# rgl-epfl/unbiased-inverse-volume-rendering

Hardware: AMD Instinct MI355X
Metric: Msamples/s primal+adjoint DRT, 256^3 grid 512^2x32spp (higher is better)
Workload: dtype f32; 1 GPU; dust-devil 256^3 sigma_t+albedo, 512x512x32spp, volpathsimple-drt, max_depth 64, majorant_resolution_factor 8 (the reference default, scene_config.py:36; with --full the global majorant is reported under other_configs.headline_global_majorant), single sensor, image tiles sharded over 1 GPU(s); spp=32, integrator=volpathsimple-drt

## Files before the change

unbiased-inverse-volume-rendering_amd/csrc/drt_capi.cpp:

```cpp
#include "../../include/drt_hip.h"
#include "drt_launch.h"

#include <hip/hip_runtime.h>

#include <cstdarg>
#include <cstdio>
#include <cmath>
#include <cstdlib>
#include <cstring>
#include <new>
#include <string>
#include <utility>
#include <vector>

using namespace drt;

#ifndef DRT_PATH_CACHE_CAP
#define DRT_PATH_CACHE_CAP 64
#endif
#ifndef DRT_ORDER_ITERS
#define DRT_ORDER_ITERS 1
#endif
#ifndef DRT_SQ_UNIT_EMPTY
#define DRT_SQ_UNIT_EMPTY 1
// ... 10 lines not shown

enum AllocMode { kMust, kBestEffort };
struct DevBuf {
    void *p = nullptr;
    size_t bytes = 0;
    DevBuf() = default;
    DevBuf(const DevBuf &) = delete;
    DevBuf &operator=(const DevBuf &) = delete;
    ~DevBuf() { release(); }
    template <class T> T *as() const { return (T *) p; }
    void release() { if (p) (void) hipFree(p); p = nullptr; bytes = 0; }
    int resize(drt_handle h, size_t need, AllocMode mode, bool wait_side = false, bool pretend_no_memory = false);
    int grow(drt_handle h, size_t need, AllocMode mode) { return need <= bytes ? DRT_OK : resize(h, need, mode); }
};

struct drt_handle_s {
    int device = 0;
    hipStream_t stream = nullptr;
    drt_config cfg{};
    drt::Params base{};
    bool have_medium = false, have_emitter = false, have_sensor = false;
    int32_t phase_kind = DRT_PHASE_ISOTROPIC;
    float *d_majorant = nullptr;
    float *h_majorant = nullptr;
    hipEvent_t ev_majorant = nullptr;
    bool majorant_pending = false;
    float majorant_seen = -1.0f;
    uint32_t *d_scratch = nullptr;
    unsigned long long *d_counters = nullptr;
    DevBuf gt;
    unsigned long long *d_queues = nullptr;
    DevBuf sq_cold;
    DevBuf uempty;
    DevBuf order;
    uint64_t order_first = 0, order_end = 0;
    uint32_t order_unit = 0;
    DevBuf tail;
    int n_cus = 256;
    DevBuf sigma_b;
    uint32_t *d_occ = nullptr;
    DevBuf mgrid;
    float *d_env = nullptr;
    DevBuf grid4;
    uint64_t grid4_version = 0;
    uint64_t medium_version = 0;
    struct RecSlot {
        DevBuf mem;
        uint64_t rays = 0;
        int bins = 0;
        bool tiny = false;
        uint32_t per_ray[2] = {0, 0};
        drt::DeferredPlan plan{};
        size_t clear_bytes = 0;
        hipEvent_t traced = nullptr, reduced = nullptr;
        bool busy = false;
    } rec[2];
    hipStream_t side = nullptr;
    const drt::DeferredPlan *early_plan = nullptr;
    bool early_done = false;
    bool early_partition = false;
    DevBuf sq_tail;
    hipEvent_t ev_split = nullptr, ev_hist = nullptr;
    hipStream_t nerf_stream = nullptr;
    hipEvent_t ev_fork = nullptr, ev_join = nullptr;
    DevBuf loss_partials;
    DevBuf dl_px;
// ... 309 lines not shown
    return DRT_OK;
}

int launch_coop(drt_handle h, const drt::Params &P, bool adjoint)
{
    drt::Params PT = P;
    no_tail(PT);
    const bool tail_pays = P.n_rays - P.ray_first >= (3u << 19) || dbg(h->debug_flags, kHookScheduleSmall);
    if (adjoint && !P.mgrid && P.n_rays > P.ray_first && tail_pays) {
        const size_t want = (((size_t) (P.n_rays - P.ray_first) / 8 + 255) / 256) * 256;
        DRT_TRY(h->tail.grow(h, want ? 256 + want * 128 : 0, kBestEffort));
        if (h->tail.p && want >= 256) {
            PT.tail_count = h->tail.as<uint32_t>(); PT.tail_pool = (uint4 *) (h->tail.as<char>() + 256); PT.tail_cap = (uint32_t) want;
        }
    }
    if (P.mgrid) {
        drt::Params Q = PT;
        Q.ray_perm = nullptr;
        DRT_HIP_CHECK(h, drt::launch_trace_coop(Q, drt::Phase::kIso, adjoint, h->counting, h->stream));
        return DRT_OK;
    }
    const bool early = adjoint && h->early_plan && PT.rec_buf[0] && PT.tail_pool && !dbg(h->debug_flags, kHookNoTailOverlap);
    if (early) {
        DRT_TRY(ensure_side_stream(h));
        DRT_TRY(ensure_event_pair(h, h->ev_split, h->ev_hist));
    }
    EarlyCtx ctx{ h, &PT };
    bool called = false;
    DRT_HIP_CHECK(h, drt::launch_trace_coop(PT, drt::Phase::kIso, adjoint, h->counting, h->stream, early ? early_histogram_between : nullptr, &ctx, &called));
    h->early_done = called;
    return DRT_OK;
}

int bind_unit_empty(drt_handle h, const drt::Params &P, drt::Params &Q)
{
    const uint64_t span = P.n_rays - P.ray_first;
    if (!(DRT_SQ_UNIT_EMPTY && P.sensor_flow && P.mocc && P.spp && span < (1ull << 31) && P.ray_first % P.spp == 0 &&
          P.ray_offset % P.spp == 0 && P.chunk % P.spp == 0 && P.stride % P.spp == 0 && !dbg(h->debug_flags, kHookWalkEmptyPixels)))
        return DRT_OK;
    const uint32_t eunits = (uint32_t) ((span + P.spp - 1) / P.spp);
    DRT_TRY(h->uempty.grow(h, eunits, kBestEffort));
    if (h->uempty.p) {
        DRT_HIP_CHECK(h, drt::build_unit_empty(P, P.spp, eunits, h->uempty.as<uint8_t>(), h->stream));
        Q.unit_empty = h->uempty.as<const uint8_t>(); Q.empty_unit = P.spp;
    }
    return DRT_OK;
}

int bind_ray_order(drt_handle h, const drt::Params &P, drt::Params &Q, bool adjoint, bool iters_ok)
{
    const uint64_t span = P.n_rays - P.ray_first;
    const uint32_t unit = P.spp >= 4u ? P.spp : 16u;
    const uint64_t min_span = dbg(h->debug_flags, kHookScheduleSmall) ? 4096u : (1u << 20);
    if (!(span >= min_span && span < (1ull << 31) && unit <= 256u && !dbg(h->debug_flags, kHookIndexOrder))) return DRT_OK;
    const uint32_t units = (uint32_t) ((span + unit - 1) / unit);
    const size_t need = drt::super_order_bytes(units);
    if (need > h->order.bytes) {
        h->order_unit = 0;
        DRT_TRY(h->order.resize(h, need, kBestEffort));
    }
    if (!h->order.p) return DRT_OK;
    const uint8_t *iters = (DRT_ORDER_ITERS && adjoint && P.path_cache_mode == 2 && iters_ok) ? P.ray_iters : nullptr;
    const bool reuse = !iters && adjoint && P.path_cache_mode == 2 && h->order_unit == unit && h->order_first == P.ray_first && h->order_end == P.n_rays;
    if (!reuse) DRT_HIP_CHECK(h, drt::build_super_order(P, unit, units, h->order.p, h->stream, iters));
    h->order_unit = (!adjoint && P.path_cache_mode == 1) || reuse ? unit : 0u;
    h->order_first = P.ray_first; h->order_end = P.n_rays;
    Q.order = h->order.as<const uint32_t>(); Q.order_unit = unit; Q.order_units = units;
    return DRT_OK;
}

int begin_supergrid_launch(drt_handle h, const drt::Params &P, drt::Params &Q, bool adjoint, const Choice &c)
{
    Q.queues = h->d_queues;
    DRT_TRY(bind_ray_order(h, P, Q, adjoint, c.route == Route::kQueued));
    Q.ray_perm = nullptr; Q.block_order = nullptr;
    if (h->majorant_pending && hipEventQuery(h->ev_majorant) == hipSuccess) { h->majorant_seen = *h->h_majorant; h->majorant_pending = false; }
    else if (h->majorant_pending) (void) hipGetLastError();
    const float dx = P.bmax[0] - P.bmin[0], dy = P.bmax[1] - P.bmin[1], dz = P.bmax[2] - P.bmin[2];
    Q.sq_rounds = (c.phase == drt::Phase::kIso && !adjoint && h->majorant_seen >= 0.0f && h->majorant_seen * std::sqrt(dx * dx + dy * dy + dz * dz) < 3.0f) ? 1u : 0u;
    DRT_HIP_CHECK(h, hipMemsetAsync(h->d_queues, 0, 8 * sizeof(unsigned long long), h->stream));
    return DRT_OK;
}

int bind_sq_tail(drt_handle h, drt::Params &Q, bool adjoint, bool hg, bool *big)
{
    const uint64_t span = Q.n_rays - Q.ray_first;
    const uint64_t tail_min = dbg(h->debug_flags, kHookScheduleSmall) ? 4096u : (1u << 21);
    *big = adjoint && h->early_plan && Q.rec_buf[0] && span >= tail_min;
    const bool solo = drt::sq_tail_solo(Q) && span >= 8192u && !*big &&
                      (adjoint ? ((DRT_SQ_TAIL_SOLO & 2) != 0 && Q.rec_buf[0] != nullptr) : (DRT_SQ_TAIL_SOLO & 1) != 0);
    const bool tail = !hg && DRT_SQ_TAIL && (*big || solo) && !dbg(h->debug_flags, kHookNoTailOverlap) && (DRT_SQ_TAIL_THIN || !Q.sq_rounds);
    if (!tail) return DRT_OK;
    const size_t cap = (size_t) h->n_cus * drt::sq_tail_push();
    DRT_TRY(h->sq_tail.grow(h, 256 + cap * drt::sq_tail_entry_quads() * sizeof(uint4), kBestEffort));
    if (!h->sq_tail.p) return DRT_OK;
    DRT_HIP_CHECK(h, hipMemsetAsync(h->sq_tail.p, 0, 256, h->stream));
    Q.tail_count = h->sq_tail.as<uint32_t>(); Q.tail_pool = (uint4 *) (h->sq_tail.as<char>() + 256); Q.tail_cap = (uint32_t) cap; Q.tail_mode = 0;
    return DRT_OK;
}

int launch_queued(drt_handle h, const drt::Params &P, bool adjoint, const Choice &c)
{
    drt::Params Q = P;
    if (adjoint && P.dL_pix) {
        const uint64_t px = (P.n_rays + P.spp - 1) / P.spp;
        DRT_TRY(h->dl_px.grow(h, (size_t) px * P.spp * 3 * sizeof(float), kMust));
        DRT_HIP_CHECK(h, drt::launch_film_backward(P.dL_pix, px, P.spp, h->dl_px.as<float>(), h->stream));
        Q.dL = h->dl_px.as<float>(); Q.dL_pix = nullptr;
    }
    DRT_TRY(bind_unit_empty(h, P, Q));
    DRT_TRY(begin_supergrid_launch(h, P, Q, adjoint, c));
    Q.sq_cold = h->sq_cold.p;
    bool big = false;
    const bool hg = c.phase != drt::Phase::kIso;
    DRT_TRY(bind_sq_tail(h, Q, adjoint, hg, &big));
    if (hg) no_tail(Q);
    DRT_HIP_CHECK(h, drt::launch_trace_sq(Q, c.phase, adjoint, h->counting, h->n_cus, h->stream));
    if (!Q.tail_pool) return DRT_OK;
    if (big) {
        DRT_TRY(ensure_side_stream(h));
        DRT_TRY(ensure_event_pair(h, h->ev_split, h->ev_hist));
        DRT_HIP_CHECK(h, hipEventRecord(h->ev_split, h->stream));
        DRT_HIP_CHECK(h, hipStreamWaitEvent(h->side, h->ev_split, 0));
        TimedSpan span;
        DRT_HIP_CHECK(h, span.begin(h, h->side));
        DRT_HIP_CHECK(h, drt::launch_deferred_reduce(Q, *h->early_plan, h->side, nullptr, false, 1));
        DRT_HIP_CHECK(h, span.end(2));
        DRT_HIP_CHECK(h, hipEventRecord(h->ev_hist, h->side));
    }
    drt::Params T = Q;
    T.tail_mode = big ? 1 : 2;
    if (big) {
        T.rec_cursor = h->sq_tail.as<uint32_t>() + 8;
        T.rec_cap_chunks[0] = T.rec_cap_chunks[1] = 0;
    }
    T.order = nullptr; T.unit_empty = nullptr;
    DRT_HIP_CHECK(h, drt::launch_trace_sq(T, c.phase, adjoint, h->counting, h->n_cus, h->stream));
    if (big) { h->early_done = true; h->early_partition = true; }
    return DRT_OK;
}

#ifdef DRT_TEST_HOOKS
int launch_older(drt_handle h, const drt::Params &P, bool adjoint, const Choice &c)
// ... 255 lines not shown
    }
    *out = h;
    return DRT_OK;
}

int drt_destroy(drt_handle h)
{
    if (!h) return DRT_OK;
    DeviceGuard g(h->device);
    for (void *p : { (void *) h->d_majorant, (void *) h->d_scratch, (void *) h->d_counters, (void *) h->d_queues, (void *) h->d_occ, (void *) h->d_env })
        if (p) (void) hipFree(p);
    if (h->h_majorant) (void) hipHostFree(h->h_majorant);
    for (hipEvent_t e : { h->ev_majorant, h->ev_fork, h->ev_join, h->ev_split, h->ev_hist, h->rec[0].traced, h->rec[0].reduced, h->rec[1].traced, h->rec[1].reduced })
        if (e) (void) hipEventDestroy(e);
    for (hipStream_t st : { h->side, h->nerf_stream })
        if (st) (void) hipStreamDestroy(st);
    clear_timings(h);
    delete h;
    return DRT_OK;
}

int drt_release_scratch(drt_handle h)
{
    if (!h) return fail(nullptr, DRT_ERR_INVALID_ARGUMENT, "null handle");
    DeviceGuard g(h->device);
    DRT_HIP_CHECK(h, hipStreamSynchronize(h->stream));
    if (h->side) DRT_HIP_CHECK(h, hipStreamSynchronize(h->side));
    for (auto &R : h->rec) {
        R.mem.release();
        R.rays = 0; R.bins = 0; R.busy = false;
    }
    h->pcache.release();
    h->pcache_sig.valid = false; h->order_valid = false; h->order_rays = 0;
    h->tail.release();
    h->dl_px.release();
    return DRT_OK;
}

int drt_set_stream(drt_handle h, void *hip_stream)
{
    if (!h) return fail(nullptr, DRT_ERR_INVALID_ARGUMENT, "null handle");
    h->stream = (hipStream_t) hip_stream;
    return DRT_OK;
}

int drt_set_ray_interleave(drt_handle h, uint64_t chunk_rays, uint64_t stride_rays)
{
    if (!h) return fail(nullptr, DRT_ERR_INVALID_ARGUMENT, "null handle");
    if (chunk_rays && stride_rays < chunk_rays)
        return fail(h, DRT_ERR_INVALID_ARGUMENT, "stride_rays must be >= chunk_rays");
    h->chunk = chunk_rays; h->stride = chunk_rays ? stride_rays : 0;
    return DRT_OK;
}

int drt_synchronize(drt_handle h)
{
    if (!h) return fail(nullptr, DRT_ERR_INVALID_ARGUMENT, "null handle");
    DeviceGuard g(h->device);
    DRT_HIP_CHECK(h, hipStreamSynchronize(h->stream));
    return DRT_OK;
}

int drt_params_changed(drt_handle h)
{
    if (!h) return fail(nullptr, DRT_ERR_INVALID_ARGUMENT, "null handle");
    h->scene_version++; h->medium_version++;
// ... 1084 lines not shown
```

unbiased-inverse-volume-rendering_amd/csrc/drt_kernels.hip:

```cpp
#include "drt_device.h"
#include "drt_launch.h"
#include "drt_coop_tracer.h"
#include "drt_nerf_kernel.h"
#include "drt_film.h"

#ifndef DRT_TRACE_WAVES
#define DRT_TRACE_WAVES 4
#endif
#ifndef DRT_XCD_RUN
#define DRT_XCD_RUN 256
#endif
namespace drt {

struct Ray { V3 o, d; float maxt; };
struct Mei { bool valid; float t; V3 p; float sigma_t; };
struct PathState { int depth; Hit si; float last_pdf; bool escaped; bool active; };

#ifdef DRT_TEST_HOOKS
template <bool COUNT, bool ENV, bool DEFER = false>
struct Tracer {
    const Params &P;
    float maj, inv_maj;
    uint32_t ray_index;
    uint32_t *rec;
// ... 634 lines not shown
    const uint32_t r = rl + batch_first * spp;
    uint32_t b = r / spp;
    Pcg32 S0; S0.seed(seed_pixels, b);
    float us = S0.next_1d(), ux = S0.next_1d(), uy = S0.next_1d();
    uint32_t si = (uint32_t)((float) n_sensors * us);
    if (si >= (uint32_t) n_sensors) si = (uint32_t) n_sensors - 1;
    const float *sn = sensors + 16 * si;
    Params P;
#pragma unroll
    for (int k = 0; k < 3; ++k) { P.cam_o[k] = sn[k]; P.cam_left[k] = sn[3 + k]; P.cam_up[k] = sn[6 + k]; P.cam_dir[k] = sn[9 + k]; }
    P.tan_x = sn[12]; P.tan_y = sn[13]; P.width = (int) sn[14]; P.height = (int) sn[15];
    uint32_t px = (uint32_t)((float) P.width * ux), py = (uint32_t)((float) P.height * uy);
    if (r == b * spp) {
        const uint32_t bl = b - batch_first;
        if (sensor_idx) sensor_idx[bl] = si;
        if (pixels) { pixels[2 * bl] = px; pixels[2 * bl + 1] = py; }
    }
    Pcg32 S1; S1.seed(seed_rays, r);
    float ox = S1.next_1d(), oy = S1.next_1d();
    V3 o, d;
    sensor_ray(P, py * (uint32_t) P.width + px, ox, oy, o, d);
    rays_o[3 * (size_t) rl] = o.x; rays_o[3 * (size_t) rl + 1] = o.y; rays_o[3 * (size_t) rl + 2] = o.z;
    rays_d[3 * (size_t) rl] = d.x; rays_d[3 * (size_t) rl + 1] = d.y; rays_d[3 * (size_t) rl + 2] = d.z;
}

__global__ void __launch_bounds__(256) film_develop_kernel(const float *L, uint64_t n_pixels, uint32_t spp, float *image)
{
    uint64_t t = (uint64_t) blockIdx.x * blockDim.x + threadIdx.x;
    if (t >= n_pixels * 3) return;
    uint64_t p = t / 3; uint32_t c = (uint32_t)(t - p * 3);
    image[t] = film_channel_sum(L, p, c, spp) * (1.0f / (float) spp);
}

__global__ void __launch_bounds__(256) film_develop_wave_kernel(const float *L, uint64_t n_pixels, uint32_t spp, float *image)
{
    const uint64_t p = (uint64_t) blockIdx.x * 4 + (threadIdx.x >> 6);
    if (p >= n_pixels) return;
    const uint32_t lane = threadIdx.x & 63u;
    float s0, s1, s2;
    film_wave_sums(L, p, spp, lane, s0, s1, s2);
    if (lane == 0) {
        const float inv = 1.0f / (float) spp;
        image[3 * p] = s0 * inv; image[3 * p + 1] = s1 * inv; image[3 * p + 2] = s2 * inv;
    }
}

__global__ void __launch_bounds__(256) film_backward_kernel(const float *grad_image, uint64_t n_pixels, uint32_t spp, float *dL)
{
    uint64_t t = (uint64_t) blockIdx.x * blockDim.x + threadIdx.x;
    if (t >= n_pixels * spp * 3) return;
    uint64_t i = t / 3; uint32_t c = (uint32_t)(t - i * 3);
    dL[t] = grad_image[3 * (i / spp) + c] * (1.0f / (float) spp);
}

__global__ void __launch_bounds__(256) debug_eval_kernel(const Params P, int op, const float *in, uint64_t n, float *out)
{
    uint64_t i = (uint64_t) blockIdx.x * blockDim.x + threadIdx.x;
    if (i >= n) return;
    const float *a = in + 6 * i;
    float *o = out + 6 * i;
    for (int k = 0; k < 6; ++k) o[k] = 0.0f;
    switch (op) {
        case 0: o[0] = drt_logf(a[0]); break;
        case 1: drt_sincos_2pi(a[0], o[0], o[1]); break;
        case 2: { V3 d = square_to_uniform_sphere(a[0], a[1]); o[0] = d.x; o[1] = d.y; o[2] = d.z; } break;
        case 3: o[0] = eval_sigma_t(P, v3(a[0], a[1], a[2]), P.occ); break;
        case 4: eval_albedo(P, v3(a[0], a[1], a[2]), o); break;
        case 5: {
            Hit h = box_hit(P, v3(a[0], a[1], a[2]), v3(a[3], a[4], a[5]));
            o[0] = h.valid ? 1.0f : 0.0f; o[1] = h.t; o[2] = h.n.x; o[3] = h.n.y; o[4] = h.n.z;
        } break;
        case 6: {
            Pcg32 S; S.seed(__float_as_uint(a[0]), __float_as_uint(a[1]));
            for (int k = 0; k < 6; ++k) o[k] = S.next_1d();
        } break;
        case 7: {
            V3 ro, rd; sensor_ray(P, __float_as_uint(a[0]), a[1], a[2], ro, rd);
            o[0] = ro.x; o[1] = ro.y; o[2] = ro.z; o[3] = rd.x; o[4] = rd.y; o[5] = rd.z;
        } break;
        case 10: o[0] = drt_expf(a[0]); break;
        case 11: o[0] = drt_atan2f(a[0], a[1]); break;
        case 12: if (P.env_pix) {
            V3 d = v3(a[0], a[1], a[2]); float Le[3];
            envmap_eval(P, d, Le); o[0] = Le[0]; o[1] = Le[1]; o[2] = Le[2]; o[3] = envmap_pdf(P, d);
        } break;
// ... 182 lines not shown
                       dim3(kUntileLanes * kUntileRows), 0, stream, P, nc, chunk);
    return hipGetLastError();
}

hipError_t launch_majorant(const float *sigma_t, size_t n, float scale, uint32_t *scratch_bits,
                           float *majorant, hipStream_t stream)
{
    hipError_t e = hipMemsetAsync(scratch_bits, 0, sizeof(uint32_t), stream);
    if (e != hipSuccess) return e;
    unsigned blocks = (unsigned) ((n + 255) / 256);
    if (blocks > 2048) blocks = 2048;
    if (blocks == 0) blocks = 1;
    hipLaunchKernelGGL(majorant_reduce_kernel, dim3(blocks), dim3(256), 0, stream, sigma_t, n, scratch_bits);
    hipLaunchKernelGGL(majorant_finalize_kernel, dim3(1), dim3(1), 0, stream, scratch_bits, scale, majorant);
    return hipGetLastError();
}

hipError_t launch_batch_raygen(const float *sensors, int n_sensors, uint32_t batch_first, uint32_t batch_size, uint32_t spp,
                               uint32_t seed_pixels, uint32_t seed_rays, float *rays_o, float *rays_d, uint32_t *sensor_idx,
                               uint32_t *pixels, hipStream_t stream)
{
    uint64_t n = (uint64_t) batch_size * spp;
    if (n == 0) return hipSuccess;
    hipLaunchKernelGGL(batch_raygen_kernel, dim3((unsigned)((n + 255) / 256)), dim3(256), 0, stream, sensors, n_sensors,
                       batch_first, batch_size, spp, seed_pixels, seed_rays, rays_o, rays_d, sensor_idx, pixels);
    return hipGetLastError();
}

hipError_t launch_film_develop(const float *L, uint64_t n_pixels, uint32_t spp, float *image, hipStream_t stream)
{
    uint64_t n = n_pixels * 3;
    if (n == 0) return hipSuccess;
    if (spp >= kFilmWaveSpp) hipLaunchKernelGGL(film_develop_wave_kernel, dim3((unsigned)((n_pixels + 3) / 4)), dim3(256), 0, stream, L, n_pixels, spp, image);
    else hipLaunchKernelGGL(film_develop_kernel, dim3((unsigned)((n + 255) / 256)), dim3(256), 0, stream, L, n_pixels, spp, image);
    return hipGetLastError();
}

__global__ void __launch_bounds__(256) adam_step_kernel(float *p, const float *g, float *m, float *v, uint64_t n,
                                                        float b1, float a1, float b2, float a2, float eps, float lr_t, float lo, float hi)
{
    const uint64_t stride = (uint64_t) gridDim.x * 256;
    const uint64_t n4 = n / 4;
    float4 *p4 = reinterpret_cast<float4 *>(p), *m4 = reinterpret_cast<float4 *>(m), *v4 = reinterpret_cast<float4 *>(v);
    const float4 *g4 = reinterpret_cast<const float4 *>(g);
    auto upd = [&](float &pp, float gg, float &mm, float &vv) {
        mm = mm * b1 + a1 * gg;
        vv = vv * b2 + a2 * (gg * gg);
        pp = pp - lr_t * (mm / (sqrtf(vv) + eps));
        pp = pp < lo ? lo : (pp > hi ? hi : pp);
    };
    for (uint64_t i = (uint64_t) blockIdx.x * 256 + threadIdx.x; i < n4; i += stride) {
        float4 P = p4[i], M = m4[i], V = v4[i]; const float4 G = g4[i];
        upd(P.x, G.x, M.x, V.x); upd(P.y, G.y, M.y, V.y); upd(P.z, G.z, M.z, V.z); upd(P.w, G.w, M.w, V.w);
        p4[i] = P; m4[i] = M; v4[i] = V;
    }
    if (blockIdx.x == 0 && threadIdx.x < (n & 3)) { const uint64_t i = n4 * 4 + threadIdx.x; upd(p[i], g[i], m[i], v[i]); }
}

hipError_t launch_adam_step(float *p, const float *g, float *m, float *v, uint64_t n, double b1, double b2, double eps, double lr_t,
                            hipStream_t stream, float lo, float hi)
{
    if (n == 0) return hipSuccess;
    const uint64_t n4 = n / 4;
    unsigned blocks = (unsigned) ((n4 + 255) / 256 < 16384 ? (n4 + 255) / 256 : 16384);
    if (blocks == 0) blocks = 1;
    hipLaunchKernelGGL(adam_step_kernel, dim3(blocks), dim3(256), 0, stream, p, g, m, v, n, (float) b1, (float) (1.0 - b1), (float) b2,
// ... 190 lines not shown
hipError_t launch_block_positions(const uint8_t *mask, uint64_t n_blocks, int32_t *pos, int32_t *count, uint32_t *group_count, hipStream_t stream)
{
    if (n_blocks == 0) return count ? hipMemsetAsync(count, 0, sizeof(int32_t), stream) : hipSuccess;
    const uint64_t n_groups = (n_blocks + kPosGroup - 1) / kPosGroup;
    if (n_groups > 0x7fffffffull) return hipErrorInvalidValue;
    hipLaunchKernelGGL(block_count_kernel, dim3((unsigned) n_groups), dim3(256), 0, stream, mask, n_blocks, group_count);
    hipLaunchKernelGGL(block_pos_kernel, dim3((unsigned) n_groups), dim3(256), 0, stream, mask, n_blocks, group_count, (uint32_t) n_groups, pos, count);
    return hipGetLastError();
}

hipError_t launch_grad_pack(float *flat, const int32_t *pos, uint64_t n_blocks, uint32_t block_floats, float *packed, float *check, bool unpack,
                            hipStream_t stream)
{
    if (n_blocks == 0) return hipSuccess;
    const uint64_t n_vec = n_blocks * (block_floats / 4);
    unsigned blocks = (unsigned) ((n_vec + 255) / 256 < 16384 ? (n_vec + 255) / 256 : 16384);
    float4 *f4 = reinterpret_cast<float4 *>(flat), *p4 = reinterpret_cast<float4 *>(packed);
#define DRT_PACK(B) do { if (unpack) hipLaunchKernelGGL((grad_pack_kernel<B, true>), dim3(blocks), dim3(256), 0, stream, f4, pos, n_vec, p4, check); \
                         else hipLaunchKernelGGL((grad_pack_kernel<B, false>), dim3(blocks), dim3(256), 0, stream, f4, pos, n_vec, p4, check); } while (0)
    switch (block_floats) {
    case 64:  DRT_PACK(64); break;
    case 128: DRT_PACK(128); break;
    case 256: DRT_PACK(256); break;
    default: return hipErrorInvalidValue;
    }
#undef DRT_PACK
    return hipGetLastError();
}

hipError_t launch_film_backward(const float *grad_image, uint64_t n_pixels, uint32_t spp, float *dL, hipStream_t stream)
{
    uint64_t n = n_pixels * spp * 3;
    if (n == 0) return hipSuccess;
    hipLaunchKernelGGL(film_backward_kernel, dim3((unsigned)((n + 255) / 256)), dim3(256), 0, stream, grad_image, n_pixels, spp, dL);
    return hipGetLastError();
}

uint32_t host_alt_seed(uint32_t seed, bool sensor_flow)
{
    Pcg32 S; S.seed(seed, 0);
    int skip = sensor_flow ? 3 : 1;
    for (int k = 0; k < skip; ++k) (void) S.next_1d();
    float u = S.next_1d();
    uint32_t bits; __builtin_memcpy(&bits, &u, 4);
    uint32_t v0, v1;
    tea32(bits, 1u, v0, v1);
    return v0;
}

}
```

unbiased-inverse-volume-rendering_amd/csrc/drt_sq_kernel.h:

```cpp
#pragma once
#include <atomic>
#include "drt_device.h"
#include "drt_launch.h"

#ifndef DRT_SQ_THREADS
#define DRT_SQ_THREADS 768
#endif
#ifndef DRT_SQ_MAX_RAYS
#define DRT_SQ_MAX_RAYS 896
#endif
#ifndef DRT_SQ_RING
#define DRT_SQ_RING 1024
#endif
#ifndef DRT_SQ_MIN_RAYS
#define DRT_SQ_MIN_RAYS 256
#endif
#ifndef DRT_SQ_K
#define DRT_SQ_K 8
#endif
#ifndef DRT_SQ_REFILL_MIN
#define DRT_SQ_REFILL_MIN 16
#endif
#ifndef DRT_SQ_BATCH
#define DRT_SQ_BATCH 56
// ... 15 lines not shown
#endif
#ifndef DRT_SQ_RT2
#define DRT_SQ_RT2 1
#endif
#ifndef DRT_SQ_PUSH_ALL
#define DRT_SQ_PUSH_ALL 1
#endif
#ifndef DRT_SQ_EARLY_OUT
#define DRT_SQ_EARLY_OUT 1
#endif
#ifndef DRT_SQ_CHUNK
#define DRT_SQ_CHUNK 256
#endif
#ifndef DRT_SQ_CHUNK_MAX
#define DRT_SQ_CHUNK_MAX 4096
#endif
#ifndef DRT_SQ_RUN
#define DRT_SQ_RUN 16384
#endif
#ifndef DRT_SQ_INLINE_K
#define DRT_SQ_INLINE_K 4
#endif
#ifndef DRT_SQ_REGEN_FINISH
#define DRT_SQ_REGEN_FINISH 2
#endif
#ifndef DRT_SQ_REGEN_AGAIN
#define DRT_SQ_REGEN_AGAIN 48
#endif
#ifndef DRT_SQ_TAIL_PUSH
#define DRT_SQ_TAIL_PUSH 64
#endif
#ifndef DRT_SQ_TAIL_BLOCKS
#define DRT_SQ_TAIL_BLOCKS 64
#endif
constexpr int kSqTailQuads = 20;
#ifndef DRT_SQ_PROFILE
#define DRT_SQ_PROFILE 0
#endif

#if DRT_SQ_PROFILE == 6
__device__ unsigned long long g_sq_dbg[160];
#endif

namespace drt {

namespace {

enum SqPhase : int {
    SP_DT = 0, SP_RT, SP_RTA, SP_DRT,
    SP_HEAD, SP_SCAT, SP_ESC, SP_NEE, SP_RT_END, SP_RTA_END, SP_PHASE, SP_END, SP_DRT_END,
    SP_IDLE, SP_NONE,
    SP_QSCAT2
};
enum SqFlight : int { SF_NEW = 0, SF_NEXT = 1, SF_WAIT = 2 };
#ifndef DRT_SQ_SPLIT
#define DRT_SQ_SPLIT 1
#endif
enum SqKind : int { SQ_WALK = 0, SQ_COLL, SQ_TA, SQ_TB, SQ_REGEN, SQ_KINDS };
constexpr uint32_t kSqEmpty = 0xffffu;
template <bool QUAD>
__device__ __forceinline__ bool sq_is_trans(int ph) { return (ph >= SP_HEAD && ph < SP_IDLE) || (QUAD && ph == SP_QSCAT2); }
template <bool SPLIT>
__device__ __forceinline__ int sq_trans_kind(int ph)
{
    if (!SPLIT) return SQ_TB;
    return (ph == SP_RT_END || ph == SP_RTA_END || ph == SP_PHASE || ph == SP_HEAD) ? SQ_TB : SQ_TA;
// ... 139 lines not shown
    const uint16_t *mg16 = (const uint16_t *) mg_lds;
    uint32_t cnt[C_COUNT];
#pragma unroll
    for (int i = 0; i < C_COUNT; ++i) cnt[i] = 0;
#if DRT_SQ_PROFILE
#define SQ_COUNT(slot) do { } while (0)
#define SQ_PROF(slot, v) do { if (DRT_SQ_PROFILE == 1 && COUNT) { const uint32_t v_ = (uint32_t) (v); if (lane == 0) cnt[slot] += v_; } } while (0)
    uint64_t pt_last = __builtin_readcyclecounter();
#define SQ_STAMP(slot) do { if (DRT_SQ_PROFILE == 2 && COUNT) { const uint64_t t_ = __builtin_readcyclecounter(); if (lane == 0) cnt[slot] += (uint32_t) ((t_ - pt_last) >> 6); pt_last = t_; } } while (0)
#define SQ_BLK(slot, pred) do { if (DRT_SQ_PROFILE >= 3 && COUNT) { const uint64_t m_ = __ballot(pred); if (m_ && lane == 0) cnt[slot] += DRT_SQ_PROFILE == 3 ? 1u : (uint32_t) __popcll(m_); } } while (0)
#else
#define SQ_STAMP(slot) do { } while (0)
#define SQ_COUNT(slot) do { if (COUNT) cnt[slot]++; } while (0)
#define SQ_PROF(slot, v) do { } while (0)
#define SQ_BLK(slot, pred) do { } while (0)
#endif

    const int gx = P.gx, gy = P.gy, gz = P.gz;
    const float fgx = (float) gx, fgy = (float) gy, fgz = (float) gz;
    const int lin_y = gx, lin_z = gx * gy;

    uint32_t *rec = recst + wave * 8;
    uint4 *cold_a = (uint4 *) P.sq_cold + (size_t) blockIdx.x * NCW * NRAY;
    uint4 *cold_b = cold_a + 3 * NRAY;
    float4 *cold_h = (float4 *) (cold_a + NC * NRAY);
    (void) cold_h;
    float2 *cold_g = (float2 *) (cold_a + (NC + 1) * NRAY);
    (void) cold_g;
    float g_acc = 0.0f;
    const uint32_t xcc = sq_xcc_id();
    const uint64_t span = P.order ? (uint64_t) P.order_units * P.order_unit : P.n_rays - P.ray_first;
    const uint64_t n_runs = (span + DRT_SQ_RUN - 1) / DRT_SQ_RUN;
    int polls = 0;
    if constexpr (TAILM) {
        {
            const uint32_t n_pool = min(*P.tail_count, P.tail_cap);
            const uint32_t n_tail = n_pool > blockIdx.x ? min((uint32_t) NRAY, (n_pool - blockIdx.x + gridDim.x - 1u) / gridDim.x) : 0u;
#pragma unroll 1
            for (uint32_t k = (uint32_t) wave; k < n_tail; k += NWV) {
                uint32_t hq;
                if (!sq_pop(ctl, SQ_REGEN, 1u, 1u, lane, hq)) break;
                uint32_t id_k = 0;
                if (lane == 0u) id_k = sq_take(q_lds, SQ_REGEN, hq);
                id_k = (uint32_t) __builtin_amdgcn_readfirstlane((int) id_k);
                const uint4 *src = P.tail_pool + ((size_t) blockIdx.x + (size_t) k * gridDim.x) * kSqTailQuads;
                uint4 v = make_uint4(0u, 0u, 0u, 0u);
                if (lane < (ADJ ? 11u + NB : 11u)) v = src[lane];
                if (lane < 7u) rec4[R4 * id_k + lane] = v;
                else if (lane >= 8u && lane < 11u) cold_a[3 * id_k + (lane - 8u)] = v;
                else if (ADJ && lane >= 11u && lane < 11u + NB) cold_b[NB * id_k + (lane - 11u)] = v;
                const int kd = __builtin_amdgcn_readlane((int) v.x, 7);
                __threadfence_block();
                sq_fence();
                sq_push(ctl, q_lds, kd, lane == 0u, id_k, lane);
            }
        }
        __syncthreads();
    }
#if DRT_SQ_PROFILE == 6
    const unsigned long long pt_start6 = __builtin_amdgcn_s_memrealtime();
#endif
#if DRT_SQ_PROFILE == 5
    const unsigned long long pt_start = __builtin_amdgcn_s_memrealtime(); unsigned long long pt_drained = 0;
#endif

    for (;;) {
    for (;;) {
        uint32_t qn = 0;
        if (lane < (uint32_t) SQ_KINDS) { const unsigned long long c = ((sq_vu64 *) ctl)[lane]; qn = (uint32_t) (c >> 32) - (uint32_t) c; }
        const uint32_t n_walk = (uint32_t) __builtin_amdgcn_readlane((int) qn, SQ_WALK), n_coll = (uint32_t) __builtin_amdgcn_readlane((int) qn, SQ_COLL);
// ... 9 lines not shown
            }
        }
#ifdef DRT_EXP_DROP_TAIL
        if (drained && (uint32_t) NRAY - dead - n_regen <= (uint32_t) DRT_EXP_DROP_TAIL) break;
#endif
#if DRT_SQ_PROFILE == 5
        if (drained && !pt_drained) pt_drained = __builtin_amdgcn_s_memrealtime();
#endif
        int kind = -1; uint32_t min_n = DRT_SQ_BATCH;
        if (n_coll >= DRT_SQ_BATCH) kind = SQ_COLL;
        else if (n_ta >= DRT_SQ_BATCH) kind = SQ_TA;
        else if (n_tb >= DRT_SQ_BATCH) kind = SQ_TB;
        else if (n_regen >= DRT_SQ_REGEN_MIN || (drained && n_regen)) { kind = SQ_REGEN; min_n = 1; }
        else if (n_walk) kind = SQ_WALK;
        else if (n_coll | n_ta | n_tb | n_regen) {
            if (polls < ((DRT_SQ_TAIL_FAST && drained) ? 0 : DRT_SQ_MAXPOLL)) { ++polls; SQ_PROF(8, 1); __builtin_amdgcn_s_sleep(4); continue; }
            const uint32_t best = max(max(n_coll, n_regen), max(n_ta, n_tb));
            kind = n_coll == best ? SQ_COLL : n_ta == best ? SQ_TA : n_tb == best ? SQ_TB : SQ_REGEN;
            min_n = 1;
        } else { SQ_PROF(8, 1); if (DRT_SQ_TAIL_FAST >= 2 && drained) __builtin_amdgcn_s_sleep(1); else __builtin_amdgcn_s_sleep(8); continue; }

        SQ_STAMP(8);
        if (kind == SQ_WALK) {
            bool fly = false, walked = false;
            uint32_t slot = 0;
            float tnx = kInf, tny = kInf, tnz = kInf, tdx = kInf, tdy = kInf, tdz = kInf, t = 0.0f, acc = 0.0f, tau = 0.0f, tmax = 0.0f;
            int cell = 0, sx = 0, sy = 0, sz = 0;
            uint32_t rem = 0;
            for (;;) {
                const uint64_t flym = __ballot(fly);
                const int nfree = 64 - __popcll(flym);
                if (nfree >= DRT_SQ_REFILL_MIN) {
                    uint32_t h0;
                    const uint32_t got = sq_pop(ctl, SQ_WALK, (uint32_t) nfree, 1u, lane, h0);
                    if (got) {
                        const uint32_t frank = (uint32_t) __popcll(~flym & ((1ull << lane) - 1ull));
                        if (!fly && frank < got) {
                            slot = sq_take(q_lds, SQ_WALK, h0 + frank);
                            const uint4 *sp = rec4 + R4 * slot;
                            const uint4 q0 = sp[0], q1 = sp[1], q2 = sp[2];
                            tnx = __uint_as_float(q0.x); tny = __uint_as_float(q0.y); tnz = __uint_as_float(q0.z); cell = (int) q0.w;
                            tdx = __uint_as_float(q1.x); tdy = __uint_as_float(q1.y); tdz = __uint_as_float(q1.z); rem = q1.w;
                            tau = __uint_as_float(q2.x); tmax = __uint_as_float(q2.y); t = __uint_as_float(q2.z); acc = __uint_as_float(q2.w);
                            sx = (rem & (1u << 27)) ? -1 : 1; sy = (rem & (1u << 28)) ? -lin_y : lin_y; sz = (rem & (1u << 29)) ? -lin_z : lin_z;
                            fly = true;
                        }
                    }
                }
                if (!__ballot(fly)) break;
                walked = true;
                SQ_STAMP(1);
                constexpr bool kLoose = !ADJ || MG;
                bool fin = false; float res_mc = 0.0f, res_t = 0.0f, res_acc = 0.0f;
#pragma unroll
                for (int k = 0; k < DRT_SQ_K; ++k) {
#if DRT_SQ_PROFILE == 1
                    { const int nf = __popcll(__ballot(fly)); SQ_PROF(0, nf); SQ_PROF(1, 1); }
#endif
                    const float tmin = fminf(fminf(tnx, tny), tnz);
                    const float texit = fminf(tmin, tmax);
                    const uint32_t ci = kLoose ? min((uint32_t) cell, (uint32_t) (n_cells - 1)) : (uint32_t) cell;
                    float mc;
                    if constexpr (MG) mc = ((mg_lds[ci >> 5] >> (ci & 31u)) & 1u) ? P.mgrid[ci] : 0.0f;
                    else mc = __uint_as_float((uint32_t) mg16[ci] << 16);
                    const float nacc = acc + mc * (texit - t);
                    const bool hit = mc > 0.0f && nacc >= tau;
                    const bool isx = tnx == tmin, isy = !isx && tny == tmin;
// ... 21 lines not shown
                SQ_STAMP(0);
                if (__ballot(fin)) {
                    if (fin) {
                        uint4 *sp = rec4 + R4 * slot;
                        sp[0].x = __float_as_uint(res_mc);
                        sp[2].z = __float_as_uint(kLoose ? res_t : t); sp[2].w = __float_as_uint(kLoose ? res_acc : acc);
                    }
                    sq_fence();
                    sq_push(ctl, q_lds, SQ_COLL, fin, slot, lane);
                }
                const int nfly = __popcll(__ballot(fly));
                if (nfly <= DRT_SQ_LEAVE_MAX) {
                    uint32_t hn = 0;
                    if (lane >= (uint32_t) SQ_COLL && lane < (uint32_t) SQ_KINDS) { const unsigned long long c = ((sq_vu64 *) ctl)[lane]; hn = (uint32_t) (c >> 32) - (uint32_t) c; }
                    if (__ballot(hn >= DRT_SQ_BATCH)) break;
                }
            }
            if (__ballot(fly)) {
                if (fly) {
                    uint4 *sp = rec4 + R4 * slot;
                    sp[0] = make_uint4(__float_as_uint(tnx), __float_as_uint(tny), __float_as_uint(tnz), (uint32_t) cell);
                    sp[1].w = rem;
                    sp[2].z = __float_as_uint(t); sp[2].w = __float_as_uint(acc);
                }
                sq_fence();
                sq_push(ctl, q_lds, SQ_WALK, fly, slot, lane);
            }
            if (walked) polls = 0;
            SQ_STAMP(1);
            continue;
        }

        uint32_t h0;
        const uint32_t nb = sq_pop(ctl, kind, 64u, min_n, lane, h0);
        if (!nb) continue;
        polls = 0;
        const bool act = lane < nb;
        uint32_t id = 0;
        if (act) id = sq_take(q_lds, kind, h0 + lane);
        sq_fence();
        uint4 *R = rec4 + R4 * id;

        int ph = SP_NONE, fl = SF_WAIT;
        bool rec_mode = false, rec_first = false, escaped = false, has_scattered = false, scat_once = false, pc_on = false;
        int depth = 0, pc_it = 0;
        uint32_t li = 0, pc_steps = 0;
        V3 ro = v3(0, 0, 0), rd = v3(0, 0, 1), wo = v3(0, 0, 0);
        float si_t = kInf, wmax = 0.0f, wt = 0.0f, nt0 = 0.0f, adjsum = 0.0f;
        float beta[3] = { 1, 1, 1 }, result[3] = { 0, 0, 0 }, dL[3] = { 0, 0, 0 };
        Pcg32 S; S.state = 0; S.inc = 1;
        Pcg32 A; A.state = 0; A.inc = 1;
        uint64_t Cst = 0;
        int r_depth = -1; float r_si_t = kInf; V3 r_o = ro, r_d = rd;
        float r_wsum[3] = { 0, 0, 0 }, r_cw[3] = { 0, 0, 0 };
        bool b_live = true;
        V3 q_ro = v3(0, 0, 0); float q_si_t = 0.0f, q_wt = 0.0f, q_result[3] = { 0, 0, 0 }; uint32_t q_flags = 0, q_sinc_lo = 1, q_sinc_hi = 0;
        bool walk_done = false;
        bool unit_empty = false;
#if DRT_SQ_PROFILE == 6
        uint32_t t_start = 0;
#endif
        float c_lm = 0.0f, c_tau = 0.0f, c_t = 0.0f, c_acc = 0.0f;
        float w_tdx = kInf, w_tdy = kInf, w_tdz = kInf; uint32_t w_rem = 0;

        if (kind != SQ_REGEN) {
            if (act) {
                const uint4 q3 = R[3], q4 = R[4], q5 = R[5], q6 = R[6];
// ... 1042 lines not shown
```

Before: 966.4 Msamples/s.

## Cache unit-empty mask across primal/adjoint, widen film kernels, spread tail work

Reuses the per-pixel empty-unit mask built in the primal pass for the matching adjoint pass, so it is not rebuilt. Adds an LDS-staged film develop kernel and a float4-store film backward kernel to cut uncoalesced memory traffic. In the tail-drain (SOLO) mode it caps how many records each wave pops, so leftover tail work is spread across more waves. Each piece is small, and the cache relies on scene_version and ray range to invalidate correctly.

```diff
diff --git a/unbiased-inverse-volume-rendering_amd/csrc/drt_capi.cpp b/unbiased-inverse-volume-rendering_amd/csrc/drt_capi.cpp
--- a/unbiased-inverse-volume-rendering_amd/csrc/drt_capi.cpp
+++ b/unbiased-inverse-volume-rendering_amd/csrc/drt_capi.cpp
@@ -66,6 +66,8 @@
     unsigned long long *d_queues = nullptr;
     DevBuf sq_cold;
     DevBuf uempty;
+    uint64_t uempty_first = 0, uempty_end = 0, uempty_version = 0;
+    uint32_t uempty_units = 0, uempty_spp = 0;
     DevBuf order;
     uint64_t order_first = 0, order_end = 0;
     uint32_t order_unit = 0;
@@ -441,18 +443,25 @@
     return DRT_OK;
 }
 
-int bind_unit_empty(drt_handle h, const drt::Params &P, drt::Params &Q)
+int bind_unit_empty(drt_handle h, const drt::Params &P, drt::Params &Q, bool adjoint)
 {
     const uint64_t span = P.n_rays - P.ray_first;
     if (!(DRT_SQ_UNIT_EMPTY && P.sensor_flow && P.mocc && P.spp && span < (1ull << 31) && P.ray_first % P.spp == 0 &&
           P.ray_offset % P.spp == 0 && P.chunk % P.spp == 0 && P.stride % P.spp == 0 && !dbg(h->debug_flags, kHookWalkEmptyPixels)))
         return DRT_OK;
     const uint32_t eunits = (uint32_t) ((span + P.spp - 1) / P.spp);
-    DRT_TRY(h->uempty.grow(h, eunits, kBestEffort));
-    if (h->uempty.p) {
+    const bool reuse = adjoint && P.path_cache_mode == 2 && h->uempty.p && h->uempty_units == eunits && h->uempty_spp == P.spp &&
+                       h->uempty_first == P.ray_first && h->uempty_end == P.n_rays && h->uempty_version == h->scene_version;
+    if (!reuse) {
+        h->uempty_units = 0;
+        DRT_TRY(h->uempty.grow(h, eunits, kBestEffort));
+        if (!h->uempty.p) return DRT_OK;
         DRT_HIP_CHECK(h, drt::build_unit_empty(P, P.spp, eunits, h->uempty.as<uint8_t>(), h->stream));
-        Q.unit_empty = h->uempty.as<const uint8_t>(); Q.empty_unit = P.spp;
-    }
+        if (!adjoint && P.path_cache_mode == 1) {
+            h->uempty_units = eunits; h->uempty_spp = P.spp; h->uempty_first = P.ray_first; h->uempty_end = P.n_rays; h->uempty_version = h->scene_version;
+        }
+    }
+    Q.unit_empty = h->uempty.as<const uint8_t>(); Q.empty_unit = P.spp;
     return DRT_OK;
 }
 
@@ -517,7 +526,7 @@
         DRT_HIP_CHECK(h, drt::launch_film_backward(P.dL_pix, px, P.spp, h->dl_px.as<float>(), h->stream));
         Q.dL = h->dl_px.as<float>(); Q.dL_pix = nullptr;
     }
-    DRT_TRY(bind_unit_empty(h, P, Q));
+    DRT_TRY(bind_unit_empty(h, P, Q, adjoint));
     DRT_TRY(begin_supergrid_launch(h, P, Q, adjoint, c));
     Q.sq_cold = h->sq_cold.p;
     bool big = false;
@@ -839,6 +848,7 @@
     }
     h->pcache.release();
     h->pcache_sig.valid = false; h->order_valid = false; h->order_rays = 0;
+    h->uempty_units = 0;
     h->tail.release();
     h->dl_px.release();
     return DRT_OK;
diff --git a/unbiased-inverse-volume-rendering_amd/csrc/drt_kernels.hip b/unbiased-inverse-volume-rendering_amd/csrc/drt_kernels.hip
--- a/unbiased-inverse-volume-rendering_amd/csrc/drt_kernels.hip
+++ b/unbiased-inverse-volume-rendering_amd/csrc/drt_kernels.hip
@@ -690,6 +690,41 @@
     image[t] = film_channel_sum(L, p, c, spp) * (1.0f / (float) spp);
 }
 
+constexpr uint32_t kFilmWideFloats = 8192;
+constexpr uint32_t kFilmWidePixels = 64;
+__global__ void __launch_bounds__(256) film_develop_wide_kernel(const float *__restrict__ L, uint64_t n_pixels, uint32_t spp, uint32_t pb,
+                                                                float *__restrict__ image)
+{
+    __shared__ float rows[kFilmWideFloats + kFilmWidePixels];
+    const uint64_t p0 = (uint64_t) blockIdx.x * pb;
+    const uint32_t np = (uint32_t) (n_pixels - p0 < (uint64_t) pb ? n_pixels - p0 : (uint64_t) pb);
+    const uint32_t rw = 3u * spp, rs = rw | 1u;
+    const uint32_t nf = np * rw, n4 = nf >> 2;
+    const float *src = L + p0 * rw;
+    for (uint32_t i = threadIdx.x; i < n4; i += 256u) {
+        const float4 v = ((const float4 *) src)[i];
+        uint32_t row = (4u * i) / rw, col = 4u * i - row * rw;
+        const float e[4] = { v.x, v.y, v.z, v.w };
+#pragma unroll
+        for (int k = 0; k < 4; ++k) {
+            rows[row * rs + col] = e[k];
+            if (++col == rw) { col = 0u; ++row; }
+        }
+    }
+    for (uint32_t f = 4u * n4 + threadIdx.x; f < nf; f += 256u) {
+        const uint32_t row = f / rw;
+        rows[row * rs + (f - row * rw)] = src[f];
+    }
+    __syncthreads();
+    for (uint32_t t = threadIdx.x; t < 3u * np; t += 256u) {
+        const uint32_t c = t / np, p = t - c * np;
+        const float *r = rows + p * rs + c;
+        float s = 0.0f;
+        for (uint32_t j = 0; j < spp; ++j) s += r[3u * j];
+        image[3 * (p0 + p) + c] = s * (1.0f / (float) spp);
+    }
+}
+
 __global__ void __launch_bounds__(256) film_develop_wave_kernel(const float *L, uint64_t n_pixels, uint32_t spp, float *image)
 {
     const uint64_t p = (uint64_t) blockIdx.x * 4 + (threadIdx.x >> 6);
@@ -709,6 +744,32 @@
     if (t >= n_pixels * spp * 3) return;
     uint64_t i = t / 3; uint32_t c = (uint32_t)(t - i * 3);
     dL[t] = grad_image[3 * (i / spp) + c] * (1.0f / (float) spp);
+}
+
+__global__ void __launch_bounds__(256) film_backward_wide_kernel(const float *__restrict__ grad_image, uint64_t n_pixels, uint32_t spp,
+                                                                 float *__restrict__ dL)
+{
+    const uint64_t n = n_pixels * spp * 3;
+    const uint64_t t0 = (uint64_t) blockIdx.x * 1024u;
+    const uint64_t i0 = t0 / 3, pix0 = i0 / spp;
+    const uint32_t c0 = (uint32_t) (t0 - 3 * i0), j0 = (uint32_t) (i0 - pix0 * spp);
+    const uint32_t o = 4u * threadIdx.x;
+    const uint64_t t = t0 + o;
+    if (t >= n) return;
+    const uint32_t u = c0 + o, di = u / 3u;
+    uint32_t c = u - 3u * di;
+    const uint32_t v = j0 + di, dp = v / spp;
+    uint32_t j = v - dp * spp;
+    uint64_t p = pix0 + dp;
+    const float inv = 1.0f / (float) spp;
+    float e[4];
+#pragma unroll
+    for (int k = 0; k < 4; ++k) {
+        e[k] = t + k < n ? grad_image[3 * p + c] * inv : 0.0f;
+        if (++c == 3u) { c = 0u; if (++j == spp) { j = 0u; ++p; } }
+    }
+    if (t + 4 <= n) *(float4 *) (dL + t) = make_float4(e[0], e[1], e[2], e[3]);
+    else for (int k = 0; k < 4 && t + k < n; ++k) dL[t + k] = e[k];
 }
 
 __global__ void __launch_bounds__(256) debug_eval_kernel(const Params P, int op, const float *in, uint64_t n, float *out)
@@ -957,6 +1018,11 @@
     uint64_t n = n_pixels * 3;
     if (n == 0) return hipSuccess;
     if (spp >= kFilmWaveSpp) hipLaunchKernelGGL(film_develop_wave_kernel, dim3((unsigned)((n_pixels + 3) / 4)), dim3(256), 0, stream, L, n_pixels, spp, image);
+    else if (((uintptr_t) L & 15u) == 0) {
+        uint32_t pb = (kFilmWideFloats / (3u * spp)) & ~3u;
+        if (pb > kFilmWidePixels) pb = kFilmWidePixels;
+        hipLaunchKernelGGL(film_develop_wide_kernel, dim3((unsigned)((n_pixels + pb - 1) / pb)), dim3(256), 0, stream, L, n_pixels, spp, pb, image);
+    }
     else hipLaunchKernelGGL(film_develop_kernel, dim3((unsigned)((n + 255) / 256)), dim3(256), 0, stream, L, n_pixels, spp, image);
     return hipGetLastError();
 }
@@ -1213,7 +1279,9 @@
 {
     uint64_t n = n_pixels * spp * 3;
     if (n == 0) return hipSuccess;
-    hipLaunchKernelGGL(film_backward_kernel, dim3((unsigned)((n + 255) / 256)), dim3(256), 0, stream, grad_image, n_pixels, spp, dL);
+    if (((uintptr_t) dL & 15u) == 0)
+        hipLaunchKernelGGL(film_backward_wide_kernel, dim3((unsigned)((n + 1023) / 1024)), dim3(256), 0, stream, grad_image, n_pixels, spp, dL);
+    else hipLaunchKernelGGL(film_backward_kernel, dim3((unsigned)((n + 255) / 256)), dim3(256), 0, stream, grad_image, n_pixels, spp, dL);
     return hipGetLastError();
 }
 
diff --git a/unbiased-inverse-volume-rendering_amd/csrc/drt_sq_kernel.h b/unbiased-inverse-volume-rendering_amd/csrc/drt_sq_kernel.h
--- a/unbiased-inverse-volume-rendering_amd/csrc/drt_sq_kernel.h
+++ b/unbiased-inverse-volume-rendering_amd/csrc/drt_sq_kernel.h
@@ -71,6 +71,9 @@
 #endif
 #ifndef DRT_SQ_TAIL_BLOCKS
 #define DRT_SQ_TAIL_BLOCKS 64
+#endif
+#ifndef DRT_SQ_TAIL_SPREAD
+#define DRT_SQ_TAIL_SPREAD 4
 #endif
 constexpr int kSqTailQuads = 20;
 #ifndef DRT_SQ_PROFILE
@@ -276,10 +279,16 @@
     const uint64_t span = P.order ? (uint64_t) P.order_units * P.order_unit : P.n_rays - P.ray_first;
     const uint64_t n_runs = (span + DRT_SQ_RUN - 1) / DRT_SQ_RUN;
     int polls = 0;
+    uint32_t tail_take = 64u;
+    (void) tail_take;
     if constexpr (TAILM) {
         {
             const uint32_t n_pool = min(*P.tail_count, P.tail_cap);
             const uint32_t n_tail = n_pool > blockIdx.x ? min((uint32_t) NRAY, (n_pool - blockIdx.x + gridDim.x - 1u) / gridDim.x) : 0u;
+            if constexpr (SOLO && DRT_SQ_TAIL_SPREAD > 0) {
+                const uint32_t share = (uint32_t) __builtin_amdgcn_readfirstlane((int) ((n_tail + NWV - 1u) / NWV));
+                if (P.tail_mode == 2u) tail_take = min(64u, max(share, (uint32_t) DRT_SQ_TAIL_SPREAD));
+            }
 #pragma unroll 1
             for (uint32_t k = (uint32_t) wave; k < n_tail; k += NWV) {
                 uint32_t hq;
@@ -355,7 +364,12 @@
                 const int nfree = 64 - __popcll(flym);
                 if (nfree >= DRT_SQ_REFILL_MIN) {
                     uint32_t h0;
-                    const uint32_t got = sq_pop(ctl, SQ_WALK, (uint32_t) nfree, 1u, lane, h0);
+                    uint32_t want = (uint32_t) nfree;
+                    if constexpr (SOLO) {
+                        const uint32_t nfly = 64u - (uint32_t) nfree;
+                        want = nfly < tail_take ? min(want, tail_take - nfly) : 0u;
+                    }
+                    const uint32_t got = sq_pop(ctl, SQ_WALK, want, 1u, lane, h0);
                     if (got) {
                         const uint32_t frank = (uint32_t) __popcll(~flym & ((1ull << lane) - 1ull));
                         if (!fly && frank < got) {
@@ -443,7 +457,8 @@
         }
 
         uint32_t h0;
-        const uint32_t nb = sq_pop(ctl, kind, 64u, min_n, lane, h0);
+        const uint32_t max_nb = (SOLO && kind != SQ_REGEN) ? tail_take : 64u;
+        const uint32_t nb = sq_pop(ctl, kind, max_nb, SOLO ? min(min_n, max_nb) : min_n, lane, h0);
         if (!nb) continue;
         polls = 0;
         const bool act = lane < nb;
```

Measured after the change: 977.9 Msamples/s (median of 6 runs). 1.01x the previous value.
